# ZJU-FAST-Lab/Dftpav

Hardware: AMD Instinct MI355X
Metric: trajectory solves/sec (batched), 16-piece MINCO (higher is better)
Workload: dtype f64

## Files before the change

dftpav_amd/csrc/solver_ref4.hip:

```cpp
#include <hip/hip_runtime.h>
#include <cstdio>
#include <cstdlib>
#include <algorithm>

#include "ref_order_common.h"
#include "quad_common.h"

namespace dftpav {
namespace reford {

constexpr int kQLcap = 7;
#ifndef DFTPAV_Q4_WAVES_PER_EU
#define DFTPAV_Q4_WAVES_PER_EU 1
#endif
constexpr int kQ4WavesPerCU = 4 * DFTPAV_Q4_WAVES_PER_EU;

struct Q4 {
  ldsd_t xs, gs;
  ldsd_t bnd;
  ldsd_t tw;
  ldsd_t st;
  ldsd_t alpha;
  ldsd_t tl;
  ldsi_t ist;
  ldsi_t tcnt;
};
__host__ __device__ inline size_t q4_team_doubles(int mem) { return 32 + 32 + 12 + 6 + sNUM + (size_t)mem + 16 * kQLcap * 3; }
__host__ __device__ inline size_t q4_team_bytes(int mem) { return (q4_team_doubles(mem) * sizeof(double) + (iNUM + 16) * sizeof(int) + 15) & ~(size_t)15; }
__host__ __device__ inline size_t q4_shared_bytes(int N) { return ((size_t)pk_segment_doubles(N) * sizeof(double) + 15) & ~(size_t)15; }
__device__ inline void q4_carve(Q4 &q, char *team, int mem) {
  ldsd_t p = (ldsd_t)reinterpret_cast<double *>(team);
  q.xs = p; p += 32;
  q.gs = p; p += 32;
  q.bnd = p; p += 12;
  q.tw = p; p += 6;
  q.st = p; p += sNUM;
  q.alpha = p; p += mem;
  q.tl = p; p += 16 * kQLcap * 3;
  ldsi_t i = (ldsi_t)p;
  q.ist = i; i += iNUM;
  q.tcnt = i;
}

__device__ __forceinline__ double row_sum32(double p0, double p1, int n, int l) {
  double acc = row_chain16(0.0, l < n ? p0 : -0.0);
  if (n > 16) acc = row_chain16(acc, 16 + l < n ? p1 : -0.0);
  return acc;
}
template <int Q>
__device__ __forceinline__ void sweep4(ldscd_t tab, double (&bq)[12], int N, int l) {
  constexpr bool DESC = Q == 1 || Q == 3, DIV = Q == 1 || Q == 2;
  ldscd_t ip = tab + 48;
  v2d_t c[pk_size(Q) / 2];
  {
    const int sl = DESC ? N - 1 - l : l;
    const int bi = sl >= 1 && sl <= N - 2 ? sl - 1 : 0;
    const ldscv2_t a = (ldscv2_t)(ip + bi * pk_size(Q));
    if (N > 2) {
#pragma unroll
      for (int u = 0; u < pk_size(Q) / 2; u++) c[u] = a[u];
    } else {
#pragma unroll
      for (int u = 0; u < pk_size(Q) / 2; u++) c[u] = v2d_t{0.0, 0.0};
    }
  }
#pragma unroll 1
  for (int s = 0; s < N; s++) {
    const int p = DESC ? N - 1 - s : s;
    double w[6][2];
#pragma unroll
    for (int r = 0; r < 6; r++)
#pragma unroll
      for (int d = 0; d < 2; d++) {
        w[r][d] = DESC ? nb_dpp<0x101>(bq[2 * (5 - r) + d]) : nb_dpp<0x111>(bq[2 * r + d]);
      }
    if (s == 0 || s == N - 1) {
      const ldscv2_t a = (ldscv2_t)(s == 0 ? tab : ip + (N - 2) * pk_size(Q));
      if (s == 0) {
#pragma unroll
        for (int r = 0; r < 6; r++) w[r][0] = w[r][1] = 0.0;
      }
      if (l == p) {
#pragma unroll
        for (int r = 0; r < 6; r++) {
          v2d_t ce[4];
#pragma unroll
          for (int u = 0; u < 4; u++) ce[u] = a[4 * r + u];
          const int rr = DESC ? 5 - r : r;
#pragma unroll
          for (int d = 0; d < 2; d++) {
            double acc = bq[2 * rr + d];
#pragma unroll
            for (int k = 0; k < 6; k++) {
              const double ck = (k & 1) ? ce[k >> 1].y : ce[k >> 1].x;
              const double t = ck * w[(r + k) % 6][d];
              acc = ck != 0.0 ? acc - t : acc;
            }
            if (DIV) acc = div_by_rcp(acc, ce[3].x, ce[3].y);
            w[r][d] = acc;
            bq[2 * rr + d] = acc;
          }
        }
      }
    } else {
      if (l == p) {
        auto at = [&](int o) { return (o & 1) ? c[o >> 1].y : c[o >> 1].x; };
#pragma unroll
        for (int r = 0; r < 6; r++) {
          const int rr = DESC ? 5 - r : r;
#pragma unroll
          for (int d = 0; d < 2; d++) {
            double acc = bq[2 * rr + d];
#pragma unroll
            for (int k = 0; k < 6; k++)
              if (pk_mask(Q, r) & (1 << k)) acc = acc - at(pk_off(Q, r, k)) * w[(r + k) % 6][d];
            if (DIV) acc = div_by_rcp(acc, at(pk_diag0(Q) + 2 * r), at(pk_diag0(Q) + 2 * r + 1));
            w[r][d] = acc;
            bq[2 * rr + d] = acc;
          }
        }
      }
    }
  }
}

__device__ __forceinline__ void q4_split(const double (&bq)[12], double (&X)[6], double (&Y)[6], int l) {
  const bool lo = (l & 8) == 0;
#pragma unroll
  for (int r = 0; r < 6; r++) {
    const double own = bq[2 * r], far = nb_dpp<0x128>(bq[2 * r + 1]);
    X[r] = lo ? own : far;
    Y[r] = lo ? far : own;
  }
}
__device__ __forceinline__ void q4_unsplit(const double (&X)[6], const double (&Y)[6], double (&bq)[12], int l) {
  const bool lo = (l & 8) == 0;
#pragma unroll
  for (int r = 0; r < 6; r++) {
    bq[2 * r] = lo ? X[r] : Y[r];
    bq[2 * r + 1] = nb_dpp<0x128>(lo ? Y[r] : X[r]);
  }
}
template <int Q>
__device__ __forceinline__ void sweep4_split(ldscd_t tab, double (&X)[6], double (&Y)[6], int l) {
  constexpr bool DESC = Q == 1 || Q == 3, DIV = Q == 1 || Q == 2;
  constexpr int N = 16;
  ldscd_t ip = tab + 48;
  const int l8 = l & 7;
  auto phase = [&](double (&R)[6], int s0, const double (&first)[6]) {
    v2d_t c[pk_size(Q) / 2];
    {
      const int sl = s0 + (DESC ? 7 - l8 : l8);
      const int bi = sl >= 1 && sl <= N - 2 ? sl - 1 : 0;
      const ldscv2_t a = (ldscv2_t)(ip + bi * pk_size(Q));
#pragma unroll
      for (int u = 0; u < pk_size(Q) / 2; u++) c[u] = a[u];
    }
#pragma unroll 1
    for (int s = s0; s < s0 + 8; s++) {
      const int p8 = (DESC ? N - 1 - s : s) & 7;
      double w[6];
#pragma unroll
      for (int r = 0; r < 6; r++) w[r] = DESC ? nb_dpp<0x101>(R[5 - r]) : nb_dpp<0x111>(R[r]);
      if (s == s0) {
#pragma unroll
        for (int r = 0; r < 6; r++) w[r] = first[r];
      }
      if (l8 != p8) continue;
      if (s == 0 || s == N - 1) {
        const ldscv2_t a = (ldscv2_t)(s == 0 ? tab : ip + (N - 2) * pk_size(Q));
#pragma unroll
        for (int r = 0; r < 6; r++) {
          v2d_t ce[4];
#pragma unroll
          for (int u = 0; u < 4; u++) ce[u] = a[4 * r + u];
          const int rr = DESC ? 5 - r : r;
          double acc = R[rr];
#pragma unroll
          for (int k = 0; k < 6; k++) {
            const double ck = (k & 1) ? ce[k >> 1].y : ce[k >> 1].x;
            const double t = ck * w[(r + k) % 6];
            acc = ck != 0.0 ? acc - t : acc;
          }
          if (DIV) acc = div_by_rcp(acc, ce[3].x, ce[3].y);
          w[r] = acc;
          R[rr] = acc;
        }
      } else {
        auto at = [&](int o) { return (o & 1) ? c[o >> 1].y : c[o >> 1].x; };
#pragma unroll
        for (int r = 0; r < 6; r++) {
          const int rr = DESC ? 5 - r : r;
          double acc = R[rr];
#pragma unroll
          for (int k = 0; k < 6; k++)
            if (pk_mask(Q, r) & (1 << k)) acc = acc - at(pk_off(Q, r, k)) * w[(r + k) % 6];
          if (DIV) acc = div_by_rcp(acc, at(pk_diag0(Q) + 2 * r), at(pk_diag0(Q) + 2 * r + 1));
          w[r] = acc;
          R[rr] = acc;
        }
      }
    }
  };
  const double zeros[6] = {0.0, 0.0, 0.0, 0.0, 0.0, 0.0};
  double mid[6];
  if (!DESC) {
    phase(X, 0, zeros);
#pragma unroll
    for (int r = 0; r < 6; r++) mid[r] = nb_dpp<0x121>(X[r]);
    phase(Y, 8, mid);
  } else {
    phase(Y, 0, zeros);
#pragma unroll
    for (int r = 0; r < 6; r++) mid[r] = nb_dpp<0x12F>(Y[5 - r]);
    phase(X, 8, mid);
  }
}

struct RectSet {
  d2_t u[5];
};
__device__ __forceinline__ void load_rect(gcd2_t cor, RectSet &r) {
#pragma unroll
  for (int u = 0; u < 5; u++) r.u[u] = cor[16 * u];
}
__device__ __forceinline__ void rect_planes(const RectSet &r, double (&pl)[20]) {
  const double C = r.u[0].x, S = r.u[0].y;
  pl[0] = -S; pl[1] = C;
  pl[4] = C; pl[5] = S;
  pl[8] = S; pl[9] = -C;
  pl[12] = -C; pl[13] = -S;
#pragma unroll
  for (int k = 0; k < 4; k++) {
    pl[4 * k + 2] = r.u[1 + k].x;
    pl[4 * k + 3] = r.u[1 + k].y;
  }
#pragma unroll
  for (int u = 16; u < 20; u++) pl[u] = 0.0;
}
template <bool FAST, bool RECT>
__device__ __forceinline__ double q4_eval(const DevBatch &D, const Q4 &q, const DenseLds &dl, ldscd_t tab, gcd_t cor, size_t cpitch, gd_t ovf, int l, Prof &pr) {
  const DevLayout &L = D.L;
  const DevParams &P = D.P;
  const int N = L.Ntot, H = FAST ? 4 : L.H, nterm = 5 * H + 4, t0 = 5 * H;
  const double epis = FAST ? 0.0 : D.epis;
  const double vt = q.xs[L.x_tau0];
  const double Tr = vt > 0.0 ? ((0.5 * vt + 1.0) * vt + 1.0) + P.mini_T : 1.0 / ((0.5 * vt - 1.0) * vt + 1.0) + P.mini_T;
  const double t1 = Tr / N, t2 = t1 * t1, t3 = t2 * t1, t4 = t2 * t2, t5 = t4 * t1;
  pr.tick(10);
  double bq[12];
#pragma unroll
  for (int u = 0; u < 12; u++) bq[u] = 0.0;
  if (l == 0) {
#pragma unroll
    for (int d = 0; d < 2; d++) {
      bq[0 + d] = q.bnd[d];
      bq[2 + d] = q.bnd[2 + d] * t1;
      bq[4 + d] = q.bnd[4 + d] * t2;
    }
  }
  if (l == N - 1) {
#pragma unroll
    for (int d = 0; d < 2; d++) {
      bq[6 + d] = q.bnd[6 + d];
      bq[8 + d] = q.bnd[8 + d] * t1;
      bq[10 + d] = q.bnd[10 + d] * t2;
    }
  } else if (l < N - 1) {
    bq[10] = q.xs[2 * l];
    bq[11] = q.xs[2 * l + 1];
  }
  if (N == 16) {
    double X[6], Y[6];
    q4_split(bq, X, Y, l);
    sweep4_split<0>(tab, X, Y, l);
    sweep4_split<1>(tab + pk_sweep_offset(1, 16), X, Y, l);
    q4_unsplit(X, Y, bq, l);
  } else {
    sweep4<0>(tab, bq, N, l);
    sweep4<1>(tab + pk_sweep_offset(1, N), bq, N, l);
  }
  pr.tick(0);
  double cc[12];
  {
    const double tI[6] = {1.0 / 1.0, 1.0 / t1, 1.0 / t2, 1.0 / t3, 1.0 / t4, 1.0 / t5};
#pragma unroll
    for (int u = 0; u < 12; u++) cc[u] = bq[u] * tI[u >> 1];
    if (l == 0) {
#pragma unroll
      for (int u = 0; u < 6; u++) q.tw[u] = tI[u];
    }
  }
  double gdC[12], pE, pG;
  {
    const double *c = cc;
    const double t[6] = {1.0, t1, t2, t3, t4, t5};
    const double n33 = c[6] * c[6] + c[7] * c[7], n44 = c[8] * c[8] + c[9] * c[9], n55 = c[10] * c[10] + c[11] * c[11];
    const double d43 = c[8] * c[6] + c[9] * c[7], d53 = c[10] * c[6] + c[11] * c[7], d54 = c[10] * c[8] + c[11] * c[9];
    pE = 36.0 * n33 * t[1] + 144.0 * d43 * t[2] + 192.0 * n44 * t[3] + 240.0 * d53 * t[3] + 720.0 * d54 * t[4] + 720.0 * n55 * t[5];
    pG = 36.0 * n33 + 288.0 * d43 * t[1] + 576.0 * n44 * t[2] + 720.0 * d53 * t[2] + 2880.0 * d54 * t[3] + 3600.0 * n55 * t[4];
#pragma unroll
    for (int d = 0; d < 2; d++) {
      const double c3 = c[6 + d], c4 = c[8 + d], c5 = c[10 + d];
      gdC[10 + d] = 240.0 * c3 * t[3] + 720.0 * c4 * t[4] + 1440.0 * c5 * t[5];
      gdC[8 + d] = 144.0 * c3 * t[2] + 384.0 * c4 * t[3] + 720.0 * c5 * t[4];
      gdC[6 + d] = 72.0 * c3 * t[1] + 144.0 * c4 * t[2] + 240.0 * c5 * t[3];
      gdC[d] = 0.0;
      gdC[2 + d] = 0.0;
      gdC[4 + d] = 0.0;
    }
  }
  pr.tick(1);
  const bool piece = l < N;
  const int Kl = (l == 0 || l == N - 1) ? L.Kd : L.K;
  const int pt0 = l == 0 ? 0 : (L.Kd + 1) + (l - 1) * (L.K + 1);
  const double step = t1 / Kl;
  const int singul_ = L.singuls[0];
  double s1 = 0.0;
  int cnt = 0;
  const gd_t ovf_l = ovf + (size_t)pt0 * nterm * 3;
  double pl[20];
  RectSet rs;
  const gcd2_t rcor = (gcd2_t)cor;
  if constexpr (RECT) load_rect(rcor, rs);
  else load_planes(cor, cpitch, H, pl);
  __builtin_amdgcn_s_waitcnt(0x0F70);
  auto take = [&](const double (&r12)[12], double e0, double e1, double e2) {
#pragma unroll
    for (int u = 0; u < 12; u++) gdC[u] += r12[u];
    if (cnt < kQLcap) {
      ldsd_t e = q.tl + (l * kQLcap + cnt) * 3;
      e[0] = e0;
      e[1] = e1;
      e[2] = e2;
    } else {
      gd_t e = ovf_l + (size_t)cnt * 3;
      e[0] = e0;
      e[1] = e1;
      e[2] = e2;
    }
    cnt++;
  };
  const int lane64 = (int)(threadIdx.x & 63);
  int listed = 0;
  unsigned mine = 0u;
  const unsigned long long here = __builtin_amdgcn_ballot_w64(true);
  const int row_here[4] = {(int)(here & 1ull), (int)((here >> 16) & 1ull), (int)((here >> 32) & 1ull), (int)((here >> 48) & 1ull)};
  const int my_row = lane64 >> 4;
  const int rank = ((my_row > 0 ? row_here[0] : 0) + (my_row > 1 ? row_here[1] : 0) + (my_row > 2 ? row_here[2] : 0)) * 16 + l;
  const int n_here = 16 * (row_here[0] + row_here[1] + row_here[2] + row_here[3]);
  auto scan_here = [&](int c, int &total) {
    int v = c;
    v += __builtin_amdgcn_update_dpp(0, v, 0x111, 0xf, 0xf, false);
    v += __builtin_amdgcn_update_dpp(0, v, 0x112, 0xf, 0xf, false);
    v += __builtin_amdgcn_update_dpp(0, v, 0x114, 0xf, 0xf, false);
    v += __builtin_amdgcn_update_dpp(0, v, 0x118, 0xf, 0xf, false);
    const int t0_ = row_here[0] ? __builtin_amdgcn_readlane(v, 15) : 0, t1_ = row_here[1] ? __builtin_amdgcn_readlane(v, 31) : 0;
    const int t2_ = row_here[2] ? __builtin_amdgcn_readlane(v, 47) : 0, t3_ = row_here[3] ? __builtin_amdgcn_readlane(v, 63) : 0;
    total = t0_ + t1_ + t2_ + t3_;
    return v + (my_row > 0 ? t0_ : 0) + (my_row > 1 ? t1_ : 0) + (my_row > 2 ? t2_ : 0);
  };
  auto flush = [&]() {
    for (int first = 0; first < listed; first += n_here) {
    const int slot = first + rank;
    const bool work = slot < listed;
    const int id = dl.id[work ? slot : 0];
    const int o = id & 63, t = (id >> 6) & 63, jo = id >> 12;
    double cco[12];
#pragma unroll
    for (int u = 0; u < 12; u++) cco[u] = __shfl(cc[u], o);
    const double t1o = __shfl(t1, o);
    const int lo = o & 15;
    const int Ko = (lo == 0 || lo == N - 1) ? L.Kd : L.K;
    const double stepo = t1o / Ko;
    if (work) {
      const double nopl[20] = {0.0, 0.0, 0.0, 0.0, 0.0, 0.0, 0.0, 0.0, 0.0, 0.0, 0.0, 0.0, 0.0, 0.0, 0.0, 0.0, 0.0, 0.0, 0.0, 0.0};
      PtState ps;
      (void)point_masks<false>(P, cco, lo, N, jo, Ko, stepo, dl.s1[slot], singul_, epis, H, nopl, (gd_t) nullptr, D.sur, 0.0, 0.0, 0, 0.0, ps);
      double r_[16];
      const ldscd_t pk = dl.pl + 4 * slot;
      point_emit_pf(P, ps, t, H, t0, [&](int, double &on0, double &on1, double &q0, double &q1) { on0 = pk[0]; on1 = pk[1]; q0 = pk[2]; q1 = pk[3]; },
                    (double *)r_);
      const bool corr = t < t0;
      ldsd_t w = dl.out + 15 * slot;
#pragma unroll
      for (int u = 0; u < 13; u++) w[u] = r_[u];
      w[13] = corr ? r_[13] : -0.0;
      w[14] = corr ? -0.0 : r_[13];
    }
    }
    __builtin_amdgcn_fence(__ATOMIC_SEQ_CST, "wavefront");
    for (unsigned mm = mine; mm;) {
      const int i = __builtin_ctz(mm);
      mm &= mm - 1;
      ldscd_t w = dl.out + 15 * i;
      double r12[12];
#pragma unroll
      for (int u = 0; u < 12; u++) r12[u] = w[u];
      take(r12, w[12], w[13], w[14]);
    }
    __builtin_amdgcn_fence(__ATOMIC_SEQ_CST, "wavefront");
    listed = 0;
    mine = 0u;
  };
#pragma unroll 1
  for (int j = 0; j <= L.Kmax + 1; j++) {
    const bool extra = j > L.Kmax;
    unsigned m = 0u;
    PtState pst;
    double nx[20];
    RectSet nr;
    if constexpr (RECT) {
      load_rect(rcor + (size_t)(j < L.Kmax ? j + 1 : L.Kmax) * 80, nr);
      rect_planes(rs, pl);
    } else {
      load_planes(cor + (size_t)(j < L.Kmax ? j + 1 : L.Kmax) * 16, cpitch, H, nx);
    }
    if (piece && j <= Kl && !extra)
      m = (unsigned)point_masks<false>(P, cc, l, N, j, Kl, step, s1, singul_, epis, H, pl, (gd_t) nullptr, D.sur, 0.0, 0.0, 0, 0.0, pst);
    const double s1_pt = s1;
    s1 += step;
    [[maybe_unused]] long long emit_t0 = 0;
    if (D.prof != nullptr) {
#ifdef DFTPAV_PROF_EMIT_CYCLES
      emit_t0 = clock64();
#else
      const int pc = __builtin_popcount(m);
      int trips = 0;
      while (__builtin_amdgcn_ballot_w64(pc > trips) != 0ull) trips++;
      pr.count(11, trips);
#endif
    }
    auto plane_of = [&](int k, double &on0, double &on1, double &q0, double &q1) {
      on0 = pl[0]; on1 = pl[1]; q0 = pl[2]; q1 = pl[3];
#pragma unroll
      for (int u = 1; u < 5; u++) {
        on0 = k == u ? pl[4 * u] : on0;
        on1 = k == u ? pl[4 * u + 1] : on1;
        q0 = k == u ? pl[4 * u + 2] : q0;
        q1 = k == u ? pl[4 * u + 3] : q1;
      }
    };
    bool in_place = false;
    const int c = __builtin_popcount(m);
    const bool any = __builtin_amdgcn_ballot_w64(c != 0) != 0ull;
    int incl = 0, total = 0;
    if (any) incl = scan_here(c, total);
    if (listed > 0 && (extra || listed + total > kDense)) flush();
    if (any && total > kDense) {
      in_place = true;
    } else if (any) {
      int e = listed + incl - c;
      for (unsigned mm = m; mm;) {
        const int t = __builtin_ctz(mm);
        mm &= mm - 1;
        dl.id[e] = lane64 | (t << 6) | (j << 12);
        dl.s1[e] = s1_pt;
        if (t < t0) {
          int v = 0;
#pragma unroll
          for (int qv = 1; qv < 5; qv++) v += t >= qv * H ? 1 : 0;
          double on0, on1, q0, q1;
          plane_of(t - v * H, on0, on1, q0, q1);
          ldsd_t w = dl.pl + 4 * e;
          w[0] = on0;
          w[1] = on1;
          w[2] = q0;
          w[3] = q1;
        }
        mine |= 1u << e;
        e++;
      }
      listed += total;
    }
    if (in_place) {
      for (unsigned mm = m; mm;) {
        const int t = __builtin_ctz(mm);
        mm &= mm - 1;
        double r_[16];
        point_emit_pf(P, pst, t, H, t0, plane_of, (double *)r_);
        const bool corr = t < t0;
        double r12[12];
#pragma unroll
        for (int u = 0; u < 12; u++) r12[u] = r_[u];
        take(r12, r_[12], corr ? r_[13] : -0.0, corr ? -0.0 : r_[13]);
      }
    }
#ifdef DFTPAV_PROF_EMIT_CYCLES
    if (D.prof != nullptr) pr.count(11, clock64() - emit_t0);
#endif
    if constexpr (RECT) {
      rs = nr;
    } else {
#pragma unroll
      for (int u = 0; u < 20; u++) pl[u] = nx[u];
    }
  }
  q.tcnt[l] = piece ? cnt : 0;
  __threadfence_block();
  pr.tick(2);
  double gdT = row_chain16(0.0, piece ? pG : -0.0);
  const double en = row_chain16(0.0, piece ? pE : -0.0);
  double cost0 = 0.0, cost2 = 0.0;
  {
    int total = 0;
    for (int p = 0; p < N; p++) total += q.tcnt[p];
    pr.count(9, total);
    if (total > 0) {
      for (int p = 0; p < N; p++) {
        const int c = q.tcnt[p];
        if (__builtin_amdgcn_ballot_w64(c != 0) == 0ull) continue;
        const int pp0 = p == 0 ? 0 : (L.Kd + 1) + (p - 1) * (L.K + 1);
        const gcd_t og = (gcd_t)(ovf + (size_t)pp0 * nterm * 3);
        {
          double e[kQLcap][3];
#pragma unroll
          for (int i = 0; i < kQLcap; i++)
#pragma unroll
            for (int w = 0; w < 3; w++) e[i][w] = q.tl[(p * kQLcap + i) * 3 + w];
#pragma unroll
          for (int i = 0; i < kQLcap; i++) {
            gdT += i < c ? e[i][0] : -0.0;
            cost0 += i < c ? e[i][1] : -0.0;
            cost2 += i < c ? e[i][2] : -0.0;
          }
        }
        for (int i0 = kQLcap; i0 < c; i0 += 8) {
          double e[8][3];
#pragma unroll
          for (int u = 0; u < 8; u++) {
            const int i = i0 + u < c ? i0 + u : c - 1;
#pragma unroll
            for (int w = 0; w < 3; w++) e[u][w] = og[(size_t)i * 3 + w];
          }
#pragma unroll
          for (int u = 0; u < 8; u++) {
            if (i0 + u < c) {
              gdT += e[u][0];
              cost0 += e[u][1];
              cost2 += e[u][2];
            }
          }
        }
      }
    }
  }
  pr.tick(3);
  double pA;
  double tI[6];
#pragma unroll
  for (int u = 0; u < 6; u++) tI[u] = q.tw[u];
  {
    const double gdtInv[6] = {0.0, -1.0 * tI[2], -2.0 * tI[3], -3.0 * tI[4], -4.0 * tI[5], -5.0 * tI[5] * tI[1]};
    double acc = 0.0;
#pragma unroll
    for (int k = 0; k < 6; k++) {
      const double gdcol = gdC[2 * k] * bq[2 * k] + gdC[2 * k + 1] * bq[2 * k + 1];
      acc += gdtInv[k] * gdcol;
    }
    pA = acc;
  }
  double adj[12];
#pragma unroll
  for (int u = 0; u < 12; u++) adj[u] = gdC[u] * tI[u >> 1];
  if (N == 16) {
    double X[6], Y[6];
    q4_split(adj, X, Y, l);
    sweep4_split<2>(tab + pk_sweep_offset(2, 16), X, Y, l);
    sweep4_split<3>(tab + pk_sweep_offset(3, 16), X, Y, l);
    q4_unsplit(X, Y, adj, l);
  } else {
    sweep4<2>(tab + pk_sweep_offset(2, N), adj, N, l);
    sweep4<3>(tab + pk_sweep_offset(3, N), adj, N, l);
  }
  pr.tick(4);
  if (l < N - 1) {
    q.gs[2 * l] = adj[10];
    q.gs[2 * l + 1] = adj[11];
  }
  {
    double hv[6], tv[6];
#pragma unroll
    for (int u = 0; u < 6; u++) {
      hv[u] = q.bnd[u];
      tv[u] = q.bnd[6 + u];
    }
    const double h1 = hv[2] * adj[2] + hv[3] * adj[3];
    const double h2 = (hv[4] * adj[4] + hv[5] * adj[5]) * 2.0 * t1;
    const double g1 = tv[2] * adj[8] + tv[3] * adj[9];
    const double g2 = (tv[4] * adj[10] + tv[5] * adj[11]) * 2.0 * t1;
    gdT = row_add_lane0(gdT, h1);
    gdT = row_add_lane0(gdT, h2);
    gdT = row_chain16(gdT, l == N - 1 ? g1 : -0.0);
    gdT = row_chain16(gdT, l == N - 1 ? g2 : -0.0);
    gdT = row_chain16(gdT, piece ? pA : -0.0);
    double gdVT2Rt;
    if (vt > 0) {
      gdVT2Rt = vt + 1.0;
    } else {
      const double denSqrt = (0.5 * vt - 1.0) * vt + 1.0;
      gdVT2Rt = (1.0 - vt) / (denSqrt * denSqrt);
    }
    if (l == 0) q.gs[L.x_tau0] = (gdT / N + P.wei_time) * gdVT2Rt;
  }
  double total_smcost = 0.0, total_timecost = 0.0, penalty_cost = 0.0;
  total_smcost += en;
  penalty_cost += (cost0 + 0.0) + cost2;
  total_timecost += Tr * P.wei_time;
  __builtin_amdgcn_fence(__ATOMIC_SEQ_CST, "wavefront");
  pr.tick(5);
  return total_smcost + total_timecost + penalty_cost;
}

struct QVec {
  double xp0, xp1, gp0, gp1, d0, d1;
};

__device__ __forceinline__ bool q4_begin_iteration(const DevParams &P, const Q4 &q, QVec &v, int n, int l) {
  const bool e0 = l < n, e1 = 16 + l < n;
  v.xp0 = e0 ? q.xs[l] : 0.0;
  v.xp1 = e1 ? q.xs[16 + l] : 0.0;
  v.gp0 = e0 ? q.gs[l] : 0.0;
  v.gp1 = e1 ? q.gs[16 + l] : 0.0;
  const double dginit = row_sum32(v.gp0 * v.d0, v.gp1 * v.d1, n, l);
  const double step = q.st[sSTEP];
  if (!(step > 0.0)) {
    if (l == 0) q.ist[iRET] = -1006;
    return false;
  }
  if (0.0 < dginit) {
    if (l == 0) q.ist[iRET] = -1005;
    return false;
  }
  if (l == 0) {
    q.st[sFINIT] = q.st[sFX];
    q.st[sDGINIT] = dginit;
    q.st[sDGTEST] = P.f_dec_coeff * dginit;
    q.st[sDSTEST] = P.s_curv_coeff * dginit;
    q.st[sMU] = 0.0;
    q.st[sNU] = P.max_step;
    q.st[sSTP] = step;
    q.ist[iCOUNT] = 0;
    q.ist[iBRACKT] = 0;
    q.ist[iTOUCHED] = 0;
  }
  if (e0) q.xs[l] = v.xp0 + step * v.d0;
  if (e1) q.xs[16 + l] = v.xp1 + step * v.d1;
  return true;
}

constexpr int kQB = 8;
struct QBlk {
  d2_t a[kQB], b[kQB];
  d2_t yr[kQB];
};
typedef double __attribute__((ext_vector_type(2))) qd2_t;
template <int DIR>
__device__ __forceinline__ void q4_load_blk(QBlk &R, gcd2_t hS, gcd2_t hR, int npad, int m, int la, int lb, int &jl) {
#pragma unroll
  for (int u = 0; u < kQB; u++) {
    const gcd2_t row = hS + (size_t)jl * npad + la;
    R.a[u] = row[0];
    R.b[u] = row[16];
    R.yr[u] = hR[jl];
    if (DIR < 0) jl = jl == 0 ? m - 1 : jl - 1;
    else jl = jl == m - 1 ? 0 : jl + 1;
  }
}
__device__ __forceinline__ void q4_pin_blk(QBlk &R) {
#pragma unroll
  for (int u = 0; u < kQB; u++)
    asm volatile("" : "+v"(R.a[u].x), "+v"(R.a[u].y), "+v"(R.b[u].x), "+v"(R.b[u].y), "+v"(R.yr[u].x), "+v"(R.yr[u].y));
}
template <bool EXACT>
__device__ __forceinline__ void q4_first_steps(const QBlk &R, const Q4 &q, int i0, int bound, int m, int n, int l, bool exact, int &j, double &d0, double &d1) {
#pragma unroll
  for (int u = 0; u < kQB; u++) {
    if (i0 + u < bound) {
      j = j == 0 ? m - 1 : j - 1;
      const double dot = row_sum32(R.a[u].x * d0, R.b[u].x * d1, n, l);
      const double a = EXACT && exact ? dot / R.yr[u].x : div_by_rcp<false>(dot, R.yr[u].x, R.yr[u].y);
      if (l == 0) q.alpha[j] = a;
      const double na = -a;
      d0 = d0 + na * R.a[u].y;
      d1 = d1 + na * R.b[u].y;
    }
  }
}
template <bool EXACT>
__device__ __forceinline__ void q4_second_steps(const QBlk &R, const Q4 &q, int i0, int bound, int m, int n, int l, bool exact, int &j, double &d0, double &d1) {
#pragma unroll
  for (int u = 0; u < kQB; u++) {
    if (i0 + u < bound) {
      const double al = q.alpha[j];
      const double dot = row_sum32(R.a[u].y * d0, R.b[u].y * d1, n, l);
      const double beta = EXACT && exact ? dot / R.yr[u].x : div_by_rcp<false>(dot, R.yr[u].x, R.yr[u].y);
      const double cf = al - beta;
      d0 = d0 + cf * R.a[u].x;
      d1 = d1 + cf * R.b[u].x;
      j = j == m - 1 ? 0 : j + 1;
    }
  }
}
template <bool EXACT>
__device__ __forceinline__ void q4_two_loop(const Q4 &q, gcd2_t hS, gcd2_t hR, int npad, int m, int n, int l, int bound, int ne, bool exact, double sc0, double &d0,
                                            double &d1) {
  const int la = l, lb = 16 + l;
  QBlk A, B;
  int j = ne;
  int jl = ne == 0 ? m - 1 : ne - 1;
  q4_load_blk<-1>(A, hS, hR, npad, m, la, lb, jl);
#pragma unroll 1
  for (int i0 = 0; i0 < bound; i0 += 2 * kQB) {
    q4_pin_blk(A);
    q4_load_blk<-1>(B, hS, hR, npad, m, la, lb, jl);
    q4_first_steps<EXACT>(A, q, i0, bound, m, n, l, exact, j, d0, d1);
    q4_pin_blk(B);
    q4_load_blk<-1>(A, hS, hR, npad, m, la, lb, jl);
    q4_first_steps<EXACT>(B, q, i0 + kQB, bound, m, n, l, exact, j, d0, d1);
  }
  d0 = d0 * sc0;
  d1 = d1 * sc0;
  __builtin_amdgcn_fence(__ATOMIC_SEQ_CST, "wavefront");
  jl = j;
  q4_load_blk<+1>(A, hS, hR, npad, m, la, lb, jl);
#pragma unroll 1
  for (int i0 = 0; i0 < bound; i0 += 2 * kQB) {
    q4_pin_blk(A);
    q4_load_blk<+1>(B, hS, hR, npad, m, la, lb, jl);
    q4_second_steps<EXACT>(A, q, i0, bound, m, n, l, exact, j, d0, d1);
    q4_pin_blk(B);
    q4_load_blk<+1>(A, hS, hR, npad, m, la, lb, jl);
    q4_second_steps<EXACT>(B, q, i0 + kQB, bound, m, n, l, exact, j, d0, d1);
  }
}

__device__ __forceinline__ void q4_advance(const DevBatch &D, const Q4 &q, QVec &v, double f, gd_t hS, gd_t hR, int l, Prof &pr) {
  const DevParams &P = D.P;
  const int n = D.L.n, m = P.mem_size, npad = D.L.npad;
  const bool e0 = l < n, e1 = 16 + l < n;
  int action = kActEval;
  if (q.ist[iPHASE] == 0) {
    const double g0 = e0 ? q.gs[l] : 0.0, g1 = e1 ? q.gs[16 + l] : 0.0;
    const double x0 = e0 ? q.xs[l] : 0.0, x1 = e1 ? q.xs[16 + l] : 0.0;
    v.d0 = e0 ? -g0 : 0.0;
    v.d1 = e1 ? -g1 : 0.0;
    const double gmax = row_max16(fmax(fabs(g0), fabs(g1))), xmax = row_max16(fmax(fabs(x0), fabs(x1)));
    const double dd = row_sum32((-g0) * (-g0), (-g1) * (-g1), n, l);
    __builtin_amdgcn_fence(__ATOMIC_SEQ_CST, "wavefront");
    if (l == 0) {
      q.st[sFX] = f;
      q.st[sPF0] = f;
      q.ist[iEVALS] = 1;
      q.ist[iEND] = 0;
      q.ist[iBOUND] = 0;
      q.ist[iHISTLO] = 0;
      q.ist[iHISTHI] = 0;
      q.ist[iPHASE] = 1;
    }
    if (gmax / fmax(1.0, xmax) < P.g_epsilon) {
      if (l == 0) {
        q.ist[iRET] = 0;
        q.ist[iK] = 0;
      }
      action = kActDone;
    } else {
      if (l == 0) {
        q.st[sSTEP] = 1.0 / sqrt(dd);
        q.ist[iK] = 1;
      }
      __threadfence_block();
      if (!q4_begin_iteration(P, q, v, n, l)) action = kActDone;
    }
    if (l == 0) q.ist[iACTION] = action;
    return;
  }

  const double fx = f;
  const double finit = q.st[sFINIT];
  double stp = q.st[sSTP];
  const int count = q.ist[iCOUNT] + 1;
  int ls = 0;
  bool decided = false;
  const int evals_before = q.ist[iEVALS];
  __threadfence_block();
  if (l == 0) {
    q.st[sFX] = fx;
    q.ist[iEVALS] = evals_before + 1;
    q.ist[iCOUNT] = count;
  }
  if (isinf(fx) || isnan(fx)) {
    ls = -1012;
    decided = true;
  } else if (P.past > 0 && fabs(finit - fx) / (fabs(finit) + 1.0) < P.delta / P.past) {
    ls = count;
    decided = true;
  } else {
    double mu = q.st[sMU], nu = q.st[sNU];
    bool brackt = q.ist[iBRACKT] != 0;
    const int touched = q.ist[iTOUCHED];
    if (fx > finit + stp * q.st[sDGTEST]) {
      nu = stp;
      brackt = true;
    } else {
      const double g0 = e0 ? q.gs[l] : 0.0, g1 = e1 ? q.gs[16 + l] : 0.0;
      const double gs = row_sum32(g0 * v.d0, g1 * v.d1, n, l);
      if (gs < q.st[sDSTEST]) {
        mu = stp;
      } else {
        ls = count;
        decided = true;
      }
    }
    bool touch_now = false;
    if (!decided) {
      if (P.max_linesearch <= count) {
        ls = -1009;
        decided = true;
      } else if (brackt && (nu - mu) < P.machine_prec * nu) {
        ls = -1007;
        decided = true;
      } else {
        if (brackt) stp = 0.5 * (mu + nu);
        else stp *= 2.0;
        if (stp < P.min_step) {
          ls = -1011;
          decided = true;
        } else if (stp > P.max_step) {
          if (touched) {
            ls = -1010;
            decided = true;
          } else {
            touch_now = true;
            stp = P.max_step;
          }
        }
      }
    }
    __threadfence_block();
    if (l == 0) {
      q.st[sMU] = mu;
      q.st[sNU] = nu;
      q.ist[iBRACKT] = brackt ? 1 : 0;
      q.st[sSTP] = stp;
      if (touch_now) q.ist[iTOUCHED] = 1;
    }
    if (!decided) {
      if (e0) q.xs[l] = v.xp0 + stp * v.d0;
      if (e1) q.xs[16 + l] = v.xp1 + stp * v.d1;
      if (l == 0) q.ist[iACTION] = kActEval;
      pr.tick(6);
      return;
    }
  }
  if (l == 0) q.st[sSTEP] = stp;
  if (ls < 0) {
    if (e0) {
      q.xs[l] = v.xp0;
      q.gs[l] = v.gp0;
    }
    if (e1) {
      q.xs[16 + l] = v.xp1;
      q.gs[16 + l] = v.gp1;
    }
    if (l == 0) {
      q.ist[iRET] = ls;
      q.ist[iACTION] = kActDone;
    }
    return;
  }

  const double x0 = e0 ? q.xs[l] : 0.0, x1 = e1 ? q.xs[16 + l] : 0.0;
  const double g0 = e0 ? q.gs[l] : 0.0, g1 = e1 ? q.gs[16 + l] : 0.0;
  int k = q.ist[iK];
  {
    const double gmax = row_max16(fmax(fabs(g0), fabs(g1))), xmax = row_max16(fmax(fabs(x0), fabs(x1)));
    const int kGoOn = 12345;
    int ret = kGoOn;
    if (gmax / fmax(1.0, xmax) < P.g_epsilon) {
      ret = 0;
    } else {
      if (0 < P.past) {
        const int slot = k % P.past;
        const double pf = q.st[sPF0 + slot];
        __threadfence_block();
        if (P.past <= k) {
          const double rate = fabs(pf - fx) / fmax(1.0, fabs(fx));
          if (rate < P.delta) ret = 1;
        }
        if (ret == kGoOn && l == 0) q.st[sPF0 + slot] = fx;
      }
      if (ret == kGoOn && P.max_iterations != 0 && P.max_iterations <= k) ret = -1008;
    }
    if (ret != kGoOn) {
      if (l == 0) {
        q.ist[iRET] = ret;
        q.ist[iACTION] = kActDone;
      }
      return;
    }
  }
  ++k;
  pr.tick(6);
  const int end = q.ist[iEND];
  int bound = q.ist[iBOUND];
  __threadfence_block();
  if (l == 0) q.ist[iK] = k;

  const double sv0 = e0 ? x0 - v.xp0 : 0.0, sv1 = e1 ? x1 - v.xp1 : 0.0;
  const double yv0 = e0 ? g0 - v.gp0 : 0.0, yv1 = e1 ? g1 - v.gp1 : 0.0;
  if (e0) {
    d2_t sy;
    sy.x = sv0;
    sy.y = yv0;
    ((gd2_t)hS)[(size_t)end * npad + l] = sy;
  }
  if (e1) {
    d2_t sy;
    sy.x = sv1;
    sy.y = yv1;
    ((gd2_t)hS)[(size_t)end * npad + 16 + l] = sy;
  }
  v.d0 = e0 ? -g0 : 0.0;
  v.d1 = e1 ? -g1 : 0.0;
  const double ys = row_sum32(yv0 * sv0, yv1 * sv1, n, l);
  const double yy = row_sum32(yv0 * yv0, yv1 * yv1, n, l);
  const double ss = row_sum32(sv0 * sv0, sv1 * sv1, n, l);
  const double gpgp = row_sum32(v.gp0 * v.gp0, v.gp1 * v.gp1, n, l);
  if (l == 0) {
    d2_t yr;
    yr.x = ys;
    yr.y = 1.0 / ys;
    ((gd2_t)hR)[end] = yr;
    if (!rcp_route_ok(ys)) q.ist[iSLOWDIV] = 1;
  }
  const double cau = ss * sqrt(gpgp) * P.cautious_factor;
  pr.tick(7);
  if (ys > cau) {
    ++bound;
    bound = m < bound ? m : bound;
    const int ne = end + 1 == m ? 0 : end + 1;
    __threadfence_block();
    const bool exact = q.ist[iSLOWDIV] != 0;
    double d0 = v.d0, d1 = v.d1;
    if (__builtin_amdgcn_ballot_w64(exact) != 0ull) q4_two_loop<true>(q, (gcd2_t)hS, (gcd2_t)hR, npad, m, n, l, bound, ne, exact, ys / yy, d0, d1);
    else q4_two_loop<false>(q, (gcd2_t)hS, (gcd2_t)hR, npad, m, n, l, bound, ne, exact, ys / yy, d0, d1);
    v.d0 = e0 ? d0 : 0.0;
    v.d1 = e1 ? d1 : 0.0;
    if (l == 0) {
      q.ist[iEND] = ne;
      q.ist[iBOUND] = bound;
      long long hs = ((long long)q.ist[iHISTHI] << 32) | (unsigned int)q.ist[iHISTLO];
      hs += bound;
      q.ist[iHISTLO] = (int)(hs & 0xffffffffLL);
      q.ist[iHISTHI] = (int)(hs >> 32);
    }
  }
  if (l == 0) q.st[sSTEP] = 1.0;
  pr.tick(8);
  __threadfence_block();
  const bool ok = q4_begin_iteration(P, q, v, n, l);
  if (l == 0) q.ist[iACTION] = ok ? kActEval : kActDone;
  pr.tick(6);
}

__device__ inline void q4_state_io(const DevBatch &D, const Q4 &q, QVec &v, int b, int l, bool save) {
  const int n = D.L.n, npad = D.L.npad;
  double *rec = D.state + (size_t)b * D.state_stride;
  for (int h = 0; h < 2; h++) {
    const int e = 16 * h + l;
    if (e >= n) {
      if (!save) {
        q.xs[e] = 0.0;
        q.gs[e] = 0.0;
        if (h == 0) { v.xp0 = 0.0; v.gp0 = 0.0; v.d0 = 0.0; } else { v.xp1 = 0.0; v.gp1 = 0.0; v.d1 = 0.0; }
      }
      continue;
    }
    if (save) {
      rec[0 * npad + e] = q.xs[e];
      rec[1 * npad + e] = h == 0 ? v.xp0 : v.xp1;
      rec[2 * npad + e] = q.gs[e];
      rec[3 * npad + e] = h == 0 ? v.gp0 : v.gp1;
      rec[4 * npad + e] = h == 0 ? v.d0 : v.d1;
    } else {
      q.xs[e] = rec[0 * npad + e];
      q.gs[e] = rec[2 * npad + e];
      if (h == 0) {
        v.xp0 = rec[1 * npad + e];
        v.gp0 = rec[3 * npad + e];
        v.d0 = rec[4 * npad + e];
      } else {
        v.xp1 = rec[1 * npad + e];
        v.gp1 = rec[3 * npad + e];
        v.d1 = rec[4 * npad + e];
      }
    }
  }
  double *r2 = rec + 5 * npad;
  for (int w = l; w < sNUM; w += 16) {
    if (save) r2[w] = q.st[w];
    else q.st[w] = r2[w];
  }
  int *ri = reinterpret_cast<int *>(r2 + 24);
  for (int w = l; w < iNUM; w += 16) {
    if (save) ri[w] = q.ist[w];
    else q.ist[w] = ri[w];
  }
}

template <bool FAST, bool RECT>
__global__ void __launch_bounds__(256, DFTPAV_Q4_WAVES_PER_EU)
    ref4_kernel(const DevBatch *__restrict__ Dp, int mode, const double *__restrict__ tabs, const double *__restrict__ cor_t, double *__restrict__ scratch, int source,
                int slice, int hand) {
  extern __shared__ double lds_raw[];
  const DevBatch &D = *Dp;
  const DevLayout &L = D.L;
  const int tidb = threadIdx.x, Tb = blockDim.x, lane = tidb & 63, wv = tidb >> 6, W = Tb >> 6, row = lane >> 4, l = lane & 15;
  const int n = L.n, N = L.Ntot, H = L.H, mem = D.P.mem_size;
  Q4 q;
  q4_carve(q, reinterpret_cast<char *>(lds_raw) + q4_shared_bytes(N) + (size_t)(wv * 4 + row) * q4_team_bytes(mem), mem);
  DenseLds dl;
  q4_carve_dense(dl, reinterpret_cast<char *>(lds_raw) + q4_shared_bytes(N) + (size_t)W * 4 * q4_team_bytes(mem) + (size_t)wv * q4_dense_bytes());
  const ldscd_t tab = (ldscd_t)lds_raw;
  for (int i = tidb; i < pk_segment_doubles(N); i += Tb) ((ldsd_t)lds_raw)[i] = tabs[i];
  __syncthreads();
  const bool ring = mode == kModeSolve && (source & 1) != 0;
  const bool force_exact_div = (source & 2) != 0;
  const int nterm = 5 * H + 4, JP = L.Kmax + 1;
  const size_t cpitch = (size_t)JP * 16;
  const size_t scratch_per_traj = (size_t)L.Npts * nterm * kRec + (size_t)L.Npts * nterm;
  Prof pr;
  pr.on = false;
  pr.acc = nullptr;
  pr.last = 0;
  QVec v{0.0, 0.0, 0.0, 0.0, 0.0, 0.0};
  int b = -1;
  bool act = false, resumed = false;
  long long tick0 = 0;
  int steps = 0;

  for (int pass = 0;; pass++) {
    if (!act) {
      int id = -1;
      if (ring) {
        for (int r = 0; r < 4; r++)
          if (row == r && l == 0) id = ring_pop(D.qctl, D.queue, D.qcap);
        id = __shfl(id, lane & 48);
      } else if (pass == 0) {
        id = ((int)blockIdx.x * W + wv) * 4 + row;
        if (id >= D.B) id = -1;
      }
      if (id >= 0) {
        b = id;
        act = true;
        resumed = ring && D.sflag[b] == 1;
        if (resumed) {
          q4_state_io(D, q, v, b, l, false);
        } else {
          const double *xsrc = (mode == kModeSolve) ? D.x0 : D.x_in;
          for (int h = 0; h < 2; h++) {
            const int e = 16 * h + l;
            q.xs[e] = e < n ? xsrc[(size_t)b * n + e] : 0.0;
            q.gs[e] = 0.0;
          }
          v = QVec{0.0, 0.0, 0.0, 0.0, 0.0, 0.0};
          q.ist[l] = (l == iSLOWDIV && force_exact_div) ? 1 : 0;
        }
        if (l < 12) q.bnd[l] = l < 6 ? D.iniS[(size_t)b * 6 + l] : D.finS[(size_t)b * 6 + (l - 6)];
        tick0 = wall_clock64();
        pr.start(D.prof != nullptr && mode == kModeSolve && l == 0, D.prof + (size_t)b * 12, resumed);
        __builtin_amdgcn_fence(__ATOMIC_SEQ_CST, "wavefront");
      }
    }
    if (__builtin_amdgcn_ballot_w64(act) == 0ull) break;
    if (act) {
      const gcd_t cor = RECT ? (gcd_t)(cor_t + ((size_t)b * JP * 80 + l) * 2) : (gcd_t)(cor_t + (size_t)b * L.H * 4 * cpitch + l);
      const gd_t ovf = (gd_t)(scratch + (size_t)b * scratch_per_traj);
      const double f = q4_eval<FAST, RECT>(D, q, dl, tab, cor, cpitch, ovf, l, pr);
      if (mode == kModeEval) {
        for (int h = 0; h < 2; h++) {
          const int e = 16 * h + l;
          if (e < n) D.g_out[(size_t)b * n + e] = q.gs[e];
        }
        if (l == 0) D.f_eval[b] = f;
        act = false;
      } else {
        const gd_t hS = (gd_t)(D.histS + (size_t)b * mem * L.npad * 2);
        const gd_t hR = (gd_t)(D.histR + (size_t)b * mem * 2);
        q4_advance(D, q, v, f, hS, hR, l, pr);
        __builtin_amdgcn_fence(__ATOMIC_SEQ_CST, "wavefront");
        if (q.ist[iACTION] == kActDone) {
          for (int h = 0; h < 2; h++) {
            const int e = 16 * h + l;
            if (e < n) D.x_out[(size_t)b * n + e] = q.xs[e];
          }
          if (l == 0) {
            const double fx = q.st[sFX];
            const int ret = q.ist[iRET];
            D.f_out[b] = fx;
            D.status[b] = ret;
            D.iters[b] = q.ist[iK];
            D.evals[b] = q.ist[iEVALS];
            D.hist_sum[b] = ((long long)q.ist[iHISTHI] << 32) | (unsigned int)q.ist[iHISTLO];
            {
              double *rec = reinterpret_cast<double *>(D.records + (size_t)16 * b);
              rec[0] = fx;
              int *ri = reinterpret_cast<int *>(rec + 1);
              ri[0] = ret;
              ri[1] = q.ist[iK];
            }
            if (D.records_host != nullptr) {
              double *rh = reinterpret_cast<double *>(D.records_host + (size_t)16 * b);
              rh[0] = fx;
              int *rj = reinterpret_cast<int *>(rh + 1);
              rj[0] = ret;
              rj[1] = q.ist[iK];
            }
            D.ticks[b] = (resumed ? D.ticks[b] : 0) + (wall_clock64() - tick0);
            int ok = (ret == 0 || ret == 1 || ret == 2 || ret == -1008 || ret == -1009) ? 1 : 0;
            if (fx >= D.P.fail_cost) ok = 0;
            D.success[b] = ok;
            if (ring) {
              D.sflag[b] = 2;
              atomicSub(&D.qctl[3], 1u);
            }
          }
          act = false;
        }
      }
    }
    if (!ring) {
      if (mode == kModeEval) break;
      continue;
    }
    steps++;
    if (slice > 0 && steps >= slice) {
      steps = 0;
      const bool leave = hand > 0 && __hip_atomic_load(&D.qctl[3], __ATOMIC_RELAXED, __HIP_MEMORY_SCOPE_AGENT) <= (unsigned)hand;
      if (act) {
        q4_state_io(D, q, v, b, l, true);
        __threadfence();
        if (l == 0) {
          D.ticks[b] = (resumed ? D.ticks[b] : 0) + (wall_clock64() - tick0);
          D.sflag[b] = 1;
        }
      }
      for (int r = 0; r < 4; r++)
        if (act && row == r && l == 0) ring_push(D.qctl, D.queue, D.qcap, b);
      act = false;
      if (leave) break;
    }
  }
}

__global__ void q4_corridor_kernel(const double *__restrict__ cor, double *__restrict__ out, int B, int H4, int NptsPad, int N, int K, int Kd, int JP) {
  const size_t total = (size_t)B * H4 * JP * 16;
  for (size_t i = (size_t)blockIdx.x * blockDim.x + threadIdx.x; i < total; i += (size_t)gridDim.x * blockDim.x) {
    const int p = (int)(i & 15);
    const size_t r = i >> 4;
    const int j = (int)(r % JP);
    const size_t bc = r / JP;
    double v = 0.0;
    if (p < N) {
      const int Kp = (p == 0 || p == N - 1) ? Kd : K;
      const int pt0 = p == 0 ? 0 : (Kd + 1) + (p - 1) * (K + 1);
      if (j <= Kp) v = cor[bc * NptsPad + pt0 + j];
    }
    out[i] = v;
  }
}

__global__ void q4_rect_check_kernel(const double *__restrict__ cor, int B, int Npts, int NptsPad, int *__restrict__ flag) {
  const size_t total = (size_t)B * Npts;
  const unsigned long long sign = 0x8000000000000000ull;
  for (size_t i = (size_t)blockIdx.x * blockDim.x + threadIdx.x; i < total; i += (size_t)gridDim.x * blockDim.x) {
    const size_t b = i / Npts;
    const int pt = (int)(i % Npts);
    const double *c = cor + b * 16 * NptsPad + pt;
    unsigned long long n[4][2];
    for (int k = 0; k < 4; k++)
      for (int q = 0; q < 2; q++) n[k][q] = (unsigned long long)__double_as_longlong(c[(size_t)(4 * k + q) * NptsPad]);
    const unsigned long long C = n[1][0], S = n[1][1];
    const bool nan = (C & ~sign) > 0x7ff0000000000000ull || (S & ~sign) > 0x7ff0000000000000ull;
    const bool ok = !nan && n[0][0] == (S ^ sign) && n[0][1] == C && n[2][0] == S && n[2][1] == (C ^ sign) && n[3][0] == (C ^ sign) && n[3][1] == (S ^ sign);
    if (!ok) *flag = 1;
  }
}

__global__ void q4_corridor_rect_kernel(const double *__restrict__ cor, d2_t *__restrict__ out, int B, int NptsPad, int N, int K, int Kd, int JP) {
  const size_t total = (size_t)B * JP * 80;
  for (size_t i = (size_t)blockIdx.x * blockDim.x + threadIdx.x; i < total; i += (size_t)gridDim.x * blockDim.x) {
    const int p = (int)(i & 15);
    const int u = (int)((i >> 4) % 5);
    const size_t r = i / 80;
    const int j = (int)(r % JP);
    const size_t b = r / JP;
    d2_t v = {0.0, 0.0};
    if (p < N) {
      const int Kp = (p == 0 || p == N - 1) ? Kd : K;
      const int pt0 = p == 0 ? 0 : (Kd + 1) + (p - 1) * (K + 1);
      if (j <= Kp) {
        const int c0 = u == 0 ? 4 : 4 * (u - 1) + 2;
        const double *src = cor + (b * 16 + c0) * NptsPad + pt0 + j;
        v.x = src[0];
        v.y = src[NptsPad];
      }
    }
    out[i] = v;
  }
}

}

bool reference_order_quad_supported(const DevLayout &L, const DevParams &P, int S) {
  if (L.M != 1 || S != 0 || L.n > 32 || L.Ntot > 16 || L.Ntot < 2 || L.H < 1 || L.H > 5) return false;
  return reford::q4_shared_bytes(L.Ntot) + 4 * reford::q4_team_bytes(P.mem_size) + reford::q4_dense_bytes() <= 160 * 1024;
}
size_t reference_order_quad_corridor_doubles(const DevLayout &L, int B) { return (size_t)B * L.H * 4 * (L.Kmax + 1) * 16; }
QuadSizes reference_order_quad_sizes(const DevLayout &L, const DevParams &P) {
  return {reford::q4_shared_bytes(L.Ntot), reford::q4_team_bytes(P.mem_size) + (reford::q4_dense_bytes() + 3) / 4, reford::kQ4WavesPerCU, 768};
}
hipError_t launch_quad_corridor(const DevBatch &D, double *cor_t, bool rect, hipStream_t stream) {
  const DevLayout &L = D.L;
  const size_t total = rect ? (size_t)D.B * (L.Kmax + 1) * 80 : reference_order_quad_corridor_doubles(L, D.B);
  const int grid = (int)std::min<size_t>((total + 255) / 256, 65536);
  if (rect)
    hipLaunchKernelGGL(reford::q4_corridor_rect_kernel, dim3(grid), dim3(256), 0, stream, D.corridor, reinterpret_cast<reford::d2_t *>(cor_t), D.B, D.NptsPad, L.Ntot, L.K,
                       L.Kd, L.Kmax + 1);
  else
    hipLaunchKernelGGL(reford::q4_corridor_kernel, dim3(grid), dim3(256), 0, stream, D.corridor, cor_t, D.B, L.H * 4, D.NptsPad, L.Ntot, L.K, L.Kd, L.Kmax + 1);
  return hipGetLastError();
}
hipError_t launch_quad_rect_check(const double *corridor, int B, int Npts, int NptsPad, int *d_flag, hipStream_t stream) {
  hipError_t e = hipMemsetAsync(d_flag, 0, sizeof(int), stream);
  if (e != hipSuccess) return e;
  const size_t total = (size_t)B * Npts;
  const int grid = (int)std::min<size_t>((total + 255) / 256, 65536);
  hipLaunchKernelGGL(reford::q4_rect_check_kernel, dim3(grid), dim3(256), 0, stream, corridor, B, Npts, NptsPad, d_flag);
  return hipGetLastError();
}
QuadKernel ref4_kernel_for(bool fast, bool rect) {
  if (fast && rect) return &reford::ref4_kernel<true, true>;
  return fast ? &reford::ref4_kernel<true, false> : &reford::ref4_kernel<false, false>;
}

}
```

Measured before the change: 39080.

## Compact per-piece quadrature terms via DPP prefix scan before reduction

Replaces the shared-memory count array and serial sum over pieces with a DPP wavefront prefix scan that yields each lane's offset and the total term count. When the terms fit, each lane packs its LDS and overflow entries contiguously, and the reduction becomes a dense blocked sweep over the packed list instead of a per-piece loop with ballots. The old per-piece path is kept as a fallback when terms exceed the dense capacity. The in-place compaction depends on wavefront fences and on the DPP row-broadcast semantics being correct for the row layout.

Result: faster. 40540 (median of 6 runs) (+3.7%).

```diff
diff --git a/dftpav_amd/csrc/solver_ref4.hip b/dftpav_amd/csrc/solver_ref4.hip
--- a/dftpav_amd/csrc/solver_ref4.hip
+++ b/dftpav_amd/csrc/solver_ref4.hip
@@ -496,17 +496,89 @@
       for (int u = 0; u < 20; u++) pl[u] = nx[u];
     }
   }
-  q.tcnt[l] = piece ? cnt : 0;
-  __threadfence_block();
+  if (!piece) cnt = 0;
   pr.tick(2);
   double gdT = row_chain16(0.0, piece ? pG : -0.0);
   const double en = row_chain16(0.0, piece ? pE : -0.0);
   double cost0 = 0.0, cost2 = 0.0;
   {
-    int total = 0;
-    for (int p = 0; p < N; p++) total += q.tcnt[p];
+    int incl = cnt;
+    incl += __builtin_amdgcn_update_dpp(0, incl, 0x111, 0xf, 0xf, false);
+    incl += __builtin_amdgcn_update_dpp(0, incl, 0x112, 0xf, 0xf, false);
+    incl += __builtin_amdgcn_update_dpp(0, incl, 0x114, 0xf, 0xf, false);
+    incl += __builtin_amdgcn_update_dpp(0, incl, 0x118, 0xf, 0xf, false);
+    const int total = __builtin_amdgcn_update_dpp(0, incl, 0x15F, 0xf, 0xf, false);
+    const int prefix = incl - cnt;
+    int longest = 0;
+#pragma unroll
+    for (int r = 0; r < 4; r++) {
+      const int tr = row_here[r] ? __builtin_amdgcn_readlane(incl, 16 * r + 15) : 0;
+      longest = tr > longest ? tr : longest;
+    }
     pr.count(9, total);
-    if (total > 0) {
+    const bool spilled = __builtin_amdgcn_ballot_w64(cnt > kQLcap) != 0ull;
+    const bool dense = longest <= 16 * kQLcap;
+    if (dense) {
+      if (longest > 0) {
+        double w[kQLcap][3];
+#pragma unroll
+        for (int i = 0; i < kQLcap; i++)
+#pragma unroll
+          for (int u = 0; u < 3; u++) w[i][u] = q.tl[(l * kQLcap + i) * 3 + u];
+        __builtin_amdgcn_fence(__ATOMIC_SEQ_CST, "wavefront");
+#pragma unroll
+        for (int i = 0; i < kQLcap; i++) {
+          if (i < cnt) {
+            ldsd_t e = q.tl + (prefix + i) * 3;
+            e[0] = w[i][0];
+            e[1] = w[i][1];
+            e[2] = w[i][2];
+          }
+        }
+        if (spilled) {
+          __threadfence_block();
+          const gcd_t og = (gcd_t)ovf_l;
+          for (int i0 = kQLcap; i0 < cnt; i0 += 4) {
+            double t[4][3];
+#pragma unroll
+            for (int u = 0; u < 4; u++) {
+              const int i = i0 + u < cnt ? i0 + u : cnt - 1;
+#pragma unroll
+              for (int c = 0; c < 3; c++) t[u][c] = og[(size_t)i * 3 + c];
+            }
+#pragma unroll
+            for (int u = 0; u < 4; u++) {
+              if (i0 + u < cnt) {
+                ldsd_t e = q.tl + (prefix + i0 + u) * 3;
+                e[0] = t[u][0];
+                e[1] = t[u][1];
+                e[2] = t[u][2];
+              }
+            }
+          }
+        }
+        __builtin_amdgcn_fence(__ATOMIC_SEQ_CST, "wavefront");
+        constexpr int kBlk = 8;
+        for (int i0 = 0; i0 < longest; i0 += kBlk) {
+          double e[kBlk][3];
+#pragma unroll
+          for (int u = 0; u < kBlk; u++) {
+            const int i = i0 + u < longest ? i0 + u : longest - 1;
+#pragma unroll
+            for (int c = 0; c < 3; c++) e[u][c] = q.tl[i * 3 + c];
+          }
+#pragma unroll
+          for (int u = 0; u < kBlk; u++) {
+            const bool on = i0 + u < total;
+            gdT += on ? e[u][0] : -0.0;
+            cost0 += on ? e[u][1] : -0.0;
+            cost2 += on ? e[u][2] : -0.0;
+          }
+        }
+      }
+    } else {
+      q.tcnt[l] = cnt;
+      __threadfence_block();
       for (int p = 0; p < N; p++) {
         const int c = q.tcnt[p];
         if (__builtin_amdgcn_ballot_w64(c != 0) == 0ull) continue;
```

## Prefetch L-BFGS history early, seed newest pair from registers, bound loops by wave max

Applied to the files above, without the earlier changes.

The obstacle-plane/rect loads are issued before the boundary sweep so their latency overlaps that compute. In the L-BFGS update, older history rows are requested before the reduction sums, and the newest (s,y) pair is placed directly from registers instead of reloaded from global memory. The two-loop recursion now iterates to the maximum bound across the rows sharing the wave, skips trailing block loads, and prefetches the second loop's first block at the end of the first loop. This adds register pressure and more complex indexing around the ring buffer's wraparound.

New measurement: 39190 before, 38490 after. -1.8%, worse.

```diff
diff --git a/dftpav_amd/csrc/solver_ref4.hip b/dftpav_amd/csrc/solver_ref4.hip
--- a/dftpav_amd/csrc/solver_ref4.hip
+++ b/dftpav_amd/csrc/solver_ref4.hip
@@ -270,6 +270,11 @@
     bq[10] = q.xs[2 * l];
     bq[11] = q.xs[2 * l + 1];
   }
+  double pl[20];
+  RectSet rs;
+  const gcd2_t rcor = (gcd2_t)cor;
+  if constexpr (RECT) load_rect(rcor, rs);
+  else load_planes(cor, cpitch, H, pl);
   if (N == 16) {
     double X[6], Y[6];
     q4_split(bq, X, Y, l);
@@ -319,11 +324,6 @@
   double s1 = 0.0;
   int cnt = 0;
   const gd_t ovf_l = ovf + (size_t)pt0 * nterm * 3;
-  double pl[20];
-  RectSet rs;
-  const gcd2_t rcor = (gcd2_t)cor;
-  if constexpr (RECT) load_rect(rcor, rs);
-  else load_planes(cor, cpitch, H, pl);
   __builtin_amdgcn_s_waitcnt(0x0F70);
   auto take = [&](const double (&r12)[12], double e0, double e1, double e2) {
 #pragma unroll
@@ -702,36 +702,57 @@
     }
   }
 }
+__device__ __forceinline__ int q4_rows_max(int v) {
+  const unsigned long long here = __builtin_amdgcn_ballot_w64(true);
+  int w = 0;
+#pragma unroll
+  for (int r = 0; r < 4; r++) {
+    const int vr = __builtin_amdgcn_readlane(v, 16 * r);
+    w = ((here >> (16 * r)) & 1ull) != 0ull && vr > w ? vr : w;
+  }
+  return w;
+}
+__device__ __forceinline__ void q4_request_older(QBlk &R, gcd2_t hS, gcd2_t hR, int npad, int m, int la, int &jl) {
+  jl = jl == 0 ? m - 1 : jl - 1;
+#pragma unroll
+  for (int u = 1; u < kQB; u++) {
+    const gcd2_t row = hS + (size_t)jl * npad + la;
+    R.a[u] = row[0];
+    R.b[u] = row[16];
+    R.yr[u] = hR[jl];
+    jl = jl == 0 ? m - 1 : jl - 1;
+  }
+}
 template <bool EXACT>
-__device__ __forceinline__ void q4_two_loop(const Q4 &q, gcd2_t hS, gcd2_t hR, int npad, int m, int n, int l, int bound, int ne, bool exact, double sc0, double &d0,
-                                            double &d1) {
+__device__ __forceinline__ void q4_two_loop(const Q4 &q, QBlk &A, gcd2_t hS, gcd2_t hR, int npad, int m, int n, int l, int bound, int wmax, int ne, int jl, bool exact,
+                                            double sc0, double &d0, double &d1) {
   const int la = l, lb = 16 + l;
-  QBlk A, B;
+  QBlk B;
   int j = ne;
-  int jl = ne == 0 ? m - 1 : ne - 1;
-  q4_load_blk<-1>(A, hS, hR, npad, m, la, lb, jl);
+  int j2 = ne - bound;
+  j2 = j2 < 0 ? j2 + m : j2;
 #pragma unroll 1
-  for (int i0 = 0; i0 < bound; i0 += 2 * kQB) {
+  for (int i0 = 0; i0 < wmax; i0 += 2 * kQB) {
     q4_pin_blk(A);
-    q4_load_blk<-1>(B, hS, hR, npad, m, la, lb, jl);
+    if (i0 + kQB < wmax) q4_load_blk<-1>(B, hS, hR, npad, m, la, lb, jl);
     q4_first_steps<EXACT>(A, q, i0, bound, m, n, l, exact, j, d0, d1);
-    q4_pin_blk(B);
-    q4_load_blk<-1>(A, hS, hR, npad, m, la, lb, jl);
-    q4_first_steps<EXACT>(B, q, i0 + kQB, bound, m, n, l, exact, j, d0, d1);
+    if (i0 + kQB < wmax) q4_pin_blk(B);
+    if (i0 + 2 * kQB < wmax) q4_load_blk<-1>(A, hS, hR, npad, m, la, lb, jl);
+    else q4_load_blk<+1>(A, hS, hR, npad, m, la, lb, j2);
+    if (i0 + kQB < wmax) q4_first_steps<EXACT>(B, q, i0 + kQB, bound, m, n, l, exact, j, d0, d1);
   }
   d0 = d0 * sc0;
   d1 = d1 * sc0;
   __builtin_amdgcn_fence(__ATOMIC_SEQ_CST, "wavefront");
-  jl = j;
-  q4_load_blk<+1>(A, hS, hR, npad, m, la, lb, jl);
+  jl = j2;
 #pragma unroll 1
-  for (int i0 = 0; i0 < bound; i0 += 2 * kQB) {
+  for (int i0 = 0; i0 < wmax; i0 += 2 * kQB) {
     q4_pin_blk(A);
-    q4_load_blk<+1>(B, hS, hR, npad, m, la, lb, jl);
+    if (i0 + kQB < wmax) q4_load_blk<+1>(B, hS, hR, npad, m, la, lb, jl);
     q4_second_steps<EXACT>(A, q, i0, bound, m, n, l, exact, j, d0, d1);
-    q4_pin_blk(B);
-    q4_load_blk<+1>(A, hS, hR, npad, m, la, lb, jl);
-    q4_second_steps<EXACT>(B, q, i0 + kQB, bound, m, n, l, exact, j, d0, d1);
+    if (i0 + kQB < wmax) q4_pin_blk(B);
+    if (i0 + 2 * kQB < wmax) q4_load_blk<+1>(A, hS, hR, npad, m, la, lb, jl);
+    if (i0 + kQB < wmax) q4_second_steps<EXACT>(B, q, i0 + kQB, bound, m, n, l, exact, j, d0, d1);
   }
 }
 
@@ -923,14 +944,21 @@
   }
   v.d0 = e0 ? -g0 : 0.0;
   v.d1 = e1 ? -g1 : 0.0;
+  QBlk A;
+  int jl = end;
+  {
+    const int nb = bound + 1;
+    if (q4_rows_max(m < nb ? m : nb) > 1) q4_request_older(A, (gcd2_t)hS, (gcd2_t)hR, npad, m, l, jl);
+  }
   const double ys = row_sum32(yv0 * sv0, yv1 * sv1, n, l);
   const double yy = row_sum32(yv0 * yv0, yv1 * yv1, n, l);
   const double ss = row_sum32(sv0 * sv0, sv1 * sv1, n, l);
   const double gpgp = row_sum32(v.gp0 * v.gp0, v.gp1 * v.gp1, n, l);
+  const double rys = 1.0 / ys;
   if (l == 0) {
     d2_t yr;
     yr.x = ys;
-    yr.y = 1.0 / ys;
+    yr.y = rys;
     ((gd2_t)hR)[end] = yr;
     if (!rcp_route_ok(ys)) q.ist[iSLOWDIV] = 1;
   }
@@ -943,8 +971,12 @@
     __threadfence_block();
     const bool exact = q.ist[iSLOWDIV] != 0;
     double d0 = v.d0, d1 = v.d1;
-    if (__builtin_amdgcn_ballot_w64(exact) != 0ull) q4_two_loop<true>(q, (gcd2_t)hS, (gcd2_t)hR, npad, m, n, l, bound, ne, exact, ys / yy, d0, d1);
-    else q4_two_loop<false>(q, (gcd2_t)hS, (gcd2_t)hR, npad, m, n, l, bound, ne, exact, ys / yy, d0, d1);
+    A.a[0].x = sv0; A.a[0].y = yv0;
+    A.b[0].x = sv1; A.b[0].y = yv1;
+    A.yr[0].x = ys; A.yr[0].y = rys;
+    const int wmax = q4_rows_max(bound);
+    if (__builtin_amdgcn_ballot_w64(exact) != 0ull) q4_two_loop<true>(q, A, (gcd2_t)hS, (gcd2_t)hR, npad, m, n, l, bound, wmax, ne, jl, exact, ys / yy, d0, d1);
+    else q4_two_loop<false>(q, A, (gcd2_t)hS, (gcd2_t)hR, npad, m, n, l, bound, wmax, ne, jl, exact, ys / yy, d0, d1);
     v.d0 = e0 ? d0 : 0.0;
     v.d1 = e1 ? d1 : 0.0;
     if (l == 0) {
```
